# janbruedigam/ConstrainedControl.jl

Hardware: AMD Instinct MI355X
Metric: LQR sim steps/sec (whole node) on N-link cartpole batch (higher is better)
Workload: dtype f64; 1 GPU; lqr_cartpole_n_pendulum N=16 links (17 bodies), hanging-equilibrium LQR, Q=I R=1 horizon 10s, y0~U(-0.5,0.5) phi_i~U(-0.2,0.2); instances_per_gpu=8192, sim_steps=1000, record=True, parallelism=instances sharded x1, lanes_per_instance=32, lds_bytes_per_workgroup=40816, launches_per_rollout=1

## Files before the change

### constrainedcontrol.jl_amd/csrc/cclqr_chain.h

```cpp
#pragma once
#include "cclqr_dev.h"

#if defined(__HIP_DEVICE_COMPILE__)
#define SCHED_FENCE() __builtin_amdgcn_sched_barrier(0)
#else
#define SCHED_FENCE() ((void)0)
#endif
#if defined(__HIP_DEVICE_COMPILE__)
#define LDS_RD(L, i) (*(const volatile __attribute__((address_space(3))) double*)(const __attribute__((address_space(3))) double*)((L) + (i)))
#else
#define LDS_RD(L, i) ((L)[i])
#endif

namespace cclqr {

struct LinkC {
    double m, J[9], p1[3], p2[3], V12[6], qoc[4], axis[3];
    double dtm;
    double sxb, sxa;
    double fric;
    int flags;
    HD bool on() const { return (flags & 1) != 0; }
    HD bool has_a() const { return (flags & 2) != 0; }
    HD bool has_c() const { return (flags & 4) != 0; }
// ... 632 lines not shown
}

struct TriPlanB { TriPlan P; int merge, st; };
HD TriPlanB tri_plan_balanced(int cs, int cn, int st = 1, int fronts = 2) {
    TriPlanB B;
    B.P = tri_plan(0, cn);
    const int rest = cn - 1;
    B.merge = (fronts == 2 && rest > 0 && rest % 2 == 0) ? 1 : 0;
    if (B.merge) { B.P.nA = B.P.nB = rest / 2; B.P.steps = rest / 2; }
    if (fronts == 1) { B.P.nB = 0; B.P.nA = rest; B.P.steps = rest; }
    B.P.cs = cs; B.P.mid = cs + st * B.P.nB; B.st = st;
    return B;
}
HD int tri_scratch_S(const TriPlanB& B, const Lay& Y) { return Y.SJP + 25 * (B.P.cs + B.st); }
HD int tri_scratch_R(const TriPlanB& B, const Lay& Y) { return Y.SPJ + 25 * (B.P.cs + 1); }
struct TriCur {
    int oLL, oQL, oRhs, oTgt, oOut;
    int dblk, dvec;
    int n;
    int imerge, oScr;
    bool isy;
};
HD TriCur tri_cursor(int t, const TriPlanB& B, const Lay& Y) {
    const TriPlan& P = B.P;
    TriCur K;
    const int front = t >> 3, col = t & 7;
    const bool in = t < 16 && col < 6;
    K.n = in ? (front ? P.nB : P.nA) : 0;
    K.isy = col == 5;
    const int st = B.st;
    const int l = front ? P.cs : P.cs + st * (P.cn - 1), q = front ? l + st : l - st;
    const int cc = col < 5 ? col : 0;
    K.dblk = front ? 25 * st : -25 * st;
    K.dvec = K.isy ? (front ? 5 * st : -5 * st) : K.dblk;
    K.oLL = Y.SJJ + 25 * l;
    K.oQL = front ? Y.SJP + 25 * q : Y.SPJ + 25 * (q + 1);
    K.oRhs = K.isy ? Y.R + 5 * l : (front ? Y.SPJ + 25 * (l + 1) : Y.SJP + 25 * l) + 5 * cc;
    K.oTgt = K.isy ? Y.R + 5 * q : Y.SJJ + 25 * q + 5 * cc;
    K.oOut = K.isy ? Y.R + 5 * l : Y.SJJ + 25 * l + 5 * cc;
    K.imerge = (front && B.merge) ? P.nB - 1 : -1;
    K.oScr = K.isy ? tri_scratch_R(B, Y) : tri_scratch_S(B, Y) + 5 * cc;
    return K;
}
HD void lu5_factor(double* A) {
#pragma unroll
    for (int k = 0; k < 5; k++) {
        const double inv = fast_rcp(A[k * 5 + k]);
        A[k * 5 + k] = inv;
#pragma unroll
        for (int i = k + 1; i < 5; i++) {
            const double f = A[i * 5 + k] * inv;
            A[i * 5 + k] = f;
#pragma unroll
            for (int j = k + 1; j < 5; j++) A[i * 5 + j] -= f * A[k * 5 + j];
        }
    }
}
HD bool tri_step(TriCur& K, int i, const double* L, double* tg, double* zy, int* otg, int* oout) {
    if (i >= K.n) return false;
    double lu[25], sql[25];
#pragma unroll
    for (int cI = 0; cI < 5; cI++)
#pragma unroll
        for (int r = 0; r < 5; r++) lu[r * 5 + cI] = LDS_RD(L, K.oLL + 5 * cI + r);
#pragma unroll
    for (int r = 0; r < 5; r++) zy[r] = LDS_RD(L, K.oRhs + r);
    const bool mstep = i == K.imerge;
    double tl[5];
#pragma unroll
    for (int r = 0; r < 5; r++) tl[r] = LDS_RD(L, K.oTgt + r);
#pragma unroll
    for (int r = 0; r < 5; r++) tg[r] = mstep ? 0.0 : tl[r];
#pragma unroll
    for (int e = 0; e < 25; e++) sql[e] = LDS_RD(L, K.oQL + e);
    lu5_factor(lu);
    lu5_solve(lu, zy);
#pragma unroll
    for (int r = 0; r < 5; r++) tg[r] -= sql[r] * zy[0] + sql[5 + r] * zy[1] + sql[10 + r] * zy[2] + sql[15 + r] * zy[3] + sql[20 + r] * zy[4];
    *otg = mstep ? K.oScr : K.oTgt; *oout = K.oOut;
    K.oLL += K.dblk; K.oQL += K.dblk; K.oRhs += K.dvec; K.oTgt += K.dvec; K.oOut += K.dvec;
    return true;
}
HD void tri_step_store(double* L, int otg, int oout, const double* tg, const double* zy) {
#pragma unroll
    for (int r = 0; r < 5; r++) { L[otg + r] = tg[r]; L[oout + r] = zy[r]; }
}
template <bool SCR = true>
HD void ck_tri_mid(int t, const TriPlanB& B, const Lay& Y, double* L) {
    if (t != 0) return;
    const TriPlan& P = B.P;
    double A[25], As[25], b[5], bs[5];
    const int oS = tri_scratch_S(B, Y), oR = tri_scratch_R(B, Y);
#pragma unroll
    for (int cI = 0; cI < 5; cI++)
#pragma unroll
        for (int r = 0; r < 5; r++) A[r * 5 + cI] = LDS_RD(L, Y.SJJ + 25 * P.mid + 5 * cI + r);
#pragma unroll
    for (int cI = 0; cI < 5; cI++)
#pragma unroll
        for (int r = 0; r < 5; r++) As[r * 5 + cI] = SCR ? LDS_RD(L, oS + 5 * cI + r) : 0.0;
#pragma unroll
    for (int i = 0; i < 5; i++) b[i] = LDS_RD(L, Y.R + 5 * P.mid + i);
#pragma unroll
    for (int i = 0; i < 5; i++) bs[i] = SCR ? LDS_RD(L, oR + i) : 0.0;
    const bool merge = SCR && B.merge != 0;
#pragma unroll
    for (int i = 0; i < 5; i++) b[i] = b[i] + (merge ? bs[i] : 0.0);
#pragma unroll
    for (int e = 0; e < 25; e++) A[e] = A[e] + (merge ? As[e] : 0.0);
    lu5_factor(A);
    lu5_solve(A, b);
#pragma unroll
    for (int i = 0; i < 5; i++) L[Y.DL + 5 * P.mid + i] = b[i];
}
HD void ck_tri_back(int t, int j, const TriPlanB& B, const Lay& Y, double* L) {
    const TriPlan& P = B.P;
    const int front = t >> 3, row = t & 7;
    if (t >= 16 || row >= 5) return;
    if (j >= (front ? P.nB : P.nA)) return;
    const int l = front ? P.mid - B.st * (1 + j) : P.mid + B.st * (1 + j);
    const int nbr = front ? l + B.st : l - B.st;
    double z[5], dn[5];
#pragma unroll
    for (int cI = 0; cI < 5; cI++) { z[cI] = LDS_RD(L, Y.SJJ + 25 * l + 5 * cI + row); dn[cI] = LDS_RD(L, Y.DL + 5 * nbr + cI); }
    const double y = LDS_RD(L, Y.R + 5 * l + row);
    L[Y.DL + 5 * l + row] = y - (z[0] * dn[0] + z[1] * dn[1] + z[2] * dn[2] + z[3] * dn[3] + z[4] * dn[4]);
}

HD void tri_step_store_fold(double* L, int otg, int oout, const double* tg, const double* zy, bool last) {
    if (!last) {
#pragma unroll
        for (int r = 0; r < 5; r++) L[otg + r] = tg[r];
    }
#pragma unroll
    for (int r = 0; r < 5; r++) L[oout + r] = zy[r];
}
struct TriBack0 { double z[5], y; int l; bool on; };
HD void ck_tri_back0_load(TriBack0& Q, int t, bool done, const TriPlanB& B, const TriCur& K, const Lay& Y, const double* L) {
    const TriPlan& P = B.P;
    const int front = t >> 3, row = t & 7;
    Q.on = !done && t < 16 && row < 5 && 0 < (front ? P.nB : P.nA);
    Q.l = P.mid + (Q.on ? B.st * (1 - 2 * front) : 0);
    const int rr = row < 5 ? row : 0;
    const bool nostep = P.steps == 0;
    const int o = nostep ? K.oOut : Y.SJJ + 25 * Q.l + rr, d = nostep ? 1 : 5;
#pragma unroll
    for (int cI = 0; cI < 5; cI++) Q.z[cI] = LDS_RD(L, o + d * cI);
    Q.y = LDS_RD(L, Y.R + 5 * Q.l + rr);
}
HD void ck_tri_back0_store(const TriBack0& Q, int t, const Lay& Y, double* L, const double* dn) {
    if (Q.on) L[Y.DL + 5 * Q.l + (t & 7)] = Q.y - (Q.z[0] * dn[0] + Q.z[1] * dn[1] + Q.z[2] * dn[2] + Q.z[3] * dn[3] + Q.z[4] * dn[4]);
}

template <int W>
struct CrLane {
    static const int NS = (11 + W - 1) / W;
    int fl;
    int w;
    int oLL, oPL, oNL;
    int oRhs[NS], oA[NS], oB[NS];
    double z[NS][5];
    HD bool act() const { return (fl & 1) != 0; }
    HD bool has_n() const { return (fl & 2) != 0; }
    HD bool ok(int s) const { return (fl & (4 << s)) != 0; }
    HD int kind(int s) const { const int k = w + W * s; return (k >= 5 ? 1 : 0) + (k >= 10 ? 1 : 0); }
};
#if defined(__HIP_DEVICE_COMPILE__)
#define CR_FLAGS_FRESH(K) asm volatile("" : "+v"((K).fl), "+v"((K).w))
#else
#define CR_FLAGS_FRESH(K) ((void)0)
#endif
template <int W>
HD void cr_setup(CrLane<W>& K, int t, int cs, int n, int st, const Lay& Y, bool skip) {
    const int i = t / W;
    K.w = t - W * i;
    const int nodd = n / 2, idx = 2 * i + 1;
    const bool act = i < nodd && !skip, has_n = idx + 1 < n;
    const int l = act ? cs + st * idx : cs + st, p = l - st, nx = l + st;
    K.oLL = Y.SJJ + 25 * l;
    K.oPL = Y.SPJ + 25 * (p + 1);
    K.oNL = has_n ? Y.SJP + 25 * nx : K.oPL;
    K.fl = (act ? 1 : 0) | (has_n ? 2 : 0);
#pragma unroll
    for (int s = 0; s < CrLane<W>::NS; s++) {
        const int k = K.w + W * s;
        const int T = K.kind(s), cI = k - 5 * T;
        const bool ok = act && k < 11 && (T != 1 || has_n);
        K.fl |= ok ? (4 << s) : 0;
        const int up_l = has_n ? Y.SPJ + 25 * (l + 1) : K.oLL;
        K.oRhs[s] = T == 0 ? Y.SJP + 25 * l + 5 * cI : (T == 1 ? up_l + 5 * cI : Y.R + 5 * l);
        K.oA[s] = T == 0 ? Y.SJJ + 25 * p + 5 * cI : (T == 1 ? K.oPL + 5 * cI : Y.R + 5 * p);
        const int nn = has_n ? nx : p;
        K.oB[s] = T == 0 ? K.oNL + 5 * cI : (T == 1 ? Y.SJJ + 25 * nn + 5 * cI : Y.R + 5 * nn);
        if (!ok) { K.oRhs[s] = K.oLL; K.oA[s] = K.oLL; K.oB[s] = K.oLL; }
    }
}
template <int W>
HD void cr_phase_a(CrLane<W>& K, const double* L, double (*tA)[5]) {
    if (!K.act()) return;
    double lu[25], blk[25];
#pragma unroll
    for (int cI = 0; cI < 5; cI++)
#pragma unroll
        for (int r = 0; r < 5; r++) lu[r * 5 + cI] = LDS_RD(L, K.oLL + 5 * cI + r);
#pragma unroll
    for (int s = 0; s < CrLane<W>::NS; s++)
#pragma unroll
        for (int r = 0; r < 5; r++) K.z[s][r] = LDS_RD(L, K.oRhs[s] + r);
    lu5_factor(lu);
#pragma unroll
    for (int s = 0; s < CrLane<W>::NS; s++) lu5_solve(lu, K.z[s]);
    SCHED_FENCE();
#pragma unroll
    for (int e = 0; e < 25; e++) blk[e] = LDS_RD(L, K.oPL + e);
#pragma unroll
    for (int s = 0; s < CrLane<W>::NS; s++)
#pragma unroll
        for (int r = 0; r < 5; r++) tA[s][r] = LDS_RD(L, K.oA[s] + r);
#pragma unroll
    for (int s = 0; s < CrLane<W>::NS; s++) {
        const double* z = K.z[s];
        const double keep = K.kind(s) != 1 ? 1.0 : 0.0;
#pragma unroll
        for (int r = 0; r < 5; r++) tA[s][r] = keep * tA[s][r] - (blk[r] * z[0] + blk[5 + r] * z[1] + blk[10 + r] * z[2] + blk[15 + r] * z[3] + blk[20 + r] * z[4]);
    }
}
template <int W>
HD void cr_store_a(const CrLane<W>& K, double* L, const double (*tA)[5]) {
#pragma unroll
    for (int s = 0; s < CrLane<W>::NS; s++)
        if (K.ok(s)) {
#pragma unroll
            for (int r = 0; r < 5; r++) { L[K.oRhs[s] + r] = K.z[s][r]; L[K.oA[s] + r] = tA[s][r]; }
        }
}
template <int W>
HD void cr_phase_b(const CrLane<W>& K, const double* L, double (*tB)[5]) {
    if (!(K.act() && K.has_n())) return;
    double blk[25];
#pragma unroll
    for (int s = 0; s < CrLane<W>::NS; s++)
#pragma unroll
        for (int r = 0; r < 5; r++) tB[s][r] = LDS_RD(L, K.oB[s] + r);
#pragma unroll
    for (int e = 0; e < 25; e++) blk[e] = LDS_RD(L, K.oNL + e);
#pragma unroll
    for (int s = 0; s < CrLane<W>::NS; s++) {
        const double* z = K.z[s];
        const double keep = K.kind(s) != 0 ? 1.0 : 0.0;
#pragma unroll
        for (int r = 0; r < 5; r++) tB[s][r] = keep * tB[s][r] - (blk[r] * z[0] + blk[5 + r] * z[1] + blk[10 + r] * z[2] + blk[15 + r] * z[3] + blk[20 + r] * z[4]);
    }
}
template <int W>
HD void cr_store_b(const CrLane<W>& K, double* L, const double (*tB)[5]) {
#pragma unroll
    for (int s = 0; s < CrLane<W>::NS; s++)
        if (K.ok(s) && K.has_n()) {
#pragma unroll
            for (int r = 0; r < 5; r++) L[K.oB[s] + r] = tB[s][r];
        }
}
template <int W>
HD void cr_back(int t, int cs, int n, int st, const Lay& Y, double* L, bool skip) {
    const int i = t / W, w = t - W * i;
    const int idx = 2 * i + 1;
    if (!(i < n / 2) || skip) return;
    const int l = cs + st * idx, p = l - st, nx = l + st;
    const bool has_n = idx + 1 < n;
    double dp[5], dn[5];
#pragma unroll
    for (int cI = 0; cI < 5; cI++) { dp[cI] = LDS_RD(L, Y.DL + 5 * p + cI); const double dnx = LDS_RD(L, Y.DL + 5 * nx + cI); dn[cI] = has_n ? dnx : 0.0; }
    const int oZm = Y.SJP + 25 * l, oZp = has_n ? Y.SPJ + 25 * (l + 1) : oZm;
    double out[(5 + W - 1) / W];
#pragma unroll
    for (int q = 0; q < (5 + W - 1) / W; q++) {
        const int row = w + W * q, rr = row < 5 ? row : 0;
        double acc = LDS_RD(L, Y.R + 5 * l + rr);
#pragma unroll
        for (int cI = 0; cI < 5; cI++) { acc -= LDS_RD(L, oZm + 5 * cI + rr) * dp[cI]; const double zp = LDS_RD(L, oZp + 5 * cI + rr); acc -= (has_n ? zp : 0.0) * dn[cI]; }
        out[q] = acc;
    }
#pragma unroll
    for (int q = 0; q < (5 + W - 1) / W; q++) {
        const int row = w + W * q;
        if (row < 5) L[Y.DL + 5 * l + row] = out[q];
    }
}
#define CR_MIN_LINKS 12

HD Lay make_chain_layout(int nb) {
    Lay L;
    L.S = L.ST = L.LT = L.DS = L.XQ = L.NB = L.DTM = L.G = L.GKB = L.GVA = L.GVB = L.UJ = L.CD = L.SS = 0;
    int o = 0;
    L.SJJ = o; o += 25 * nb; L.SJP = o; o += 25 * nb; L.SPJ = o; o += 25 * nb;
    L.R = o; o += 5 * nb; L.DL = o; o += 5 * nb;
    L.GKA = o; o += GKSZ * nb;
    L.LAM = o; o += 5 * nb;
    L.DINV = o; o += 9 * nb;
    L.D = o; o += 6 * nb;
    L.C = o; o += 6 * nb;
    L.Z = L.SJJ;
    L.DZ = L.SJJ + 13 * nb;
    L.total = o | 1;
    return L;
}
// ... 14 lines not shown
```

### constrainedcontrol.jl_amd/csrc/cclqr_newton.h

```cpp
#pragma once
#include "cclqr_dev.h"

namespace cclqr {

#ifdef CCLQR_PROFILE
enum { PF_CONTROL, PF_FORCES, PF_EVAL_BODY, PF_EVAL_JOINT, PF_EVAL_MAP, PF_SCHUR_W, PF_SCHUR_S, PF_TRI_FWD, PF_TRI_BWD, PF_BODY_SOLVE, PF_TRIAL,
       PF_ACCEPT, PF_IO, PF_NEWTON_ITERS, PF_EVALS, PF_STEPS, PF_ROWS_SKIPPED, PF_N };
static __device__ unsigned long long g_prof[PF_N];
struct Prof {
    unsigned long long t0, acc[PF_N];
    __device__ void start() { for (int i = 0; i < PF_N; i++) acc[i] = 0; t0 = __builtin_readcyclecounter(); }
    __device__ void stamp(int c) { unsigned long long t1 = __builtin_readcyclecounter(); acc[c] += t1 - t0; t0 = t1; }
    __device__ void count(int c, int n = 1) { acc[c] += n; }
    __device__ void flush() { if ((threadIdx.x & 63) == 0) for (int i = 0; i < PF_N; i++) atomicAdd(&g_prof[i], acc[i]); }
};
enum { PF_READ_N = 16 };
static_assert(PF_READ_N == PF_ROWS_SKIPPED && PF_READ_N <= PF_N, "a new counter goes behind the words that two-argument readers receive");
static inline int prof_read(unsigned long long* out, int cap, int reset) {
    int n = cap < PF_N ? cap : PF_N;
    if (!out || n < 0) return -1;
    hipError_t e = hipMemcpyFromSymbol(out, HIP_SYMBOL(g_prof), sizeof(unsigned long long) * n);
    if (e == hipSuccess && reset) { unsigned long long z[PF_N] = {0}; e = hipMemcpyToSymbol(HIP_SYMBOL(g_prof), z, sizeof(z)); }
    return e == hipSuccess ? n : -1;
}
#define PROF_ARG , Prof& prof
#define PROF_PASS , prof
#define STAMP(c) prof.stamp(c)
#define PCOUNT(c) prof.count(c)
#else
#define PROF_ARG
#define PROF_PASS
#define STAMP(c)
#define PCOUNT(c)
#endif

#define NEWTON_EPS 1e-10
#define NEWTON_MAXIT 100
#define LINE_MAXIT 10

struct NewtonStatus { int worst; bool bad, dead; };
__device__ __forceinline__ NewtonStatus status_decode(int carried) {
    return {carried < 0 ? -carried : carried, carried < 0, carried < 0 && carried > -NEWTON_MAXIT};
}
__device__ __forceinline__ int status_encode(int worst, bool bad, bool dead, int carry) {
    return bad ? -((carry && dead && worst >= NEWTON_MAXIT) ? NEWTON_MAXIT - 1 : worst) : worst;
}

template <int N>
__device__ __forceinline__ double dpp_row_ror(double v) {
    int lo = __double2loint(v), hi = __double2hiint(v);
    lo = __builtin_amdgcn_update_dpp(0, lo, 0x120 + N, 0xf, 0xf, true);
    hi = __builtin_amdgcn_update_dpp(0, hi, 0x120 + N, 0xf, 0xf, true);
    return __hiloint2double(hi, lo);
}
template <int CTRL>
__device__ __forceinline__ double dpp_f64(double v) {
    int lo = __double2loint(v), hi = __double2hiint(v);
    lo = __builtin_amdgcn_update_dpp(0, lo, CTRL, 0xf, 0xf, true);
    hi = __builtin_amdgcn_update_dpp(0, hi, CTRL, 0xf, 0xf, true);
    return __hiloint2double(hi, lo);
}
template <int G>
__device__ __forceinline__ double group_sum(double v) {
    if (G == 8) {
        v += dpp_f64<0x141>(v);
        v += dpp_f64<0xB1>(v);
        v += dpp_f64<0x4E>(v);
        return v;
    }
    v += dpp_row_ror<8>(v);
    v += dpp_row_ror<4>(v);
    v += dpp_row_ror<2>(v);
    v += dpp_row_ror<1>(v);
    if (G == 32) v += __shfl_xor(v, 16, 64);
    if (G == 64) {
        int lo = __double2loint(v), hi = __double2hiint(v);
        double r0 = __hiloint2double(__builtin_amdgcn_readlane(hi, 0), __builtin_amdgcn_readlane(lo, 0));
        double r1 = __hiloint2double(__builtin_amdgcn_readlane(hi, 16), __builtin_amdgcn_readlane(lo, 16));
        double r2 = __hiloint2double(__builtin_amdgcn_readlane(hi, 32), __builtin_amdgcn_readlane(lo, 32));
        double r3 = __hiloint2double(__builtin_amdgcn_readlane(hi, 48), __builtin_amdgcn_readlane(lo, 48));
        v = (r0 + r1) + (r2 + r3);
    }
    return v;
}

__device__ __forceinline__ Lay fresh_layout(int nb) {
    asm volatile("" : "+s"(nb));
    return make_layout(nb, 0);
}
#define FRESH_Y fresh_layout(nb)
__device__ __forceinline__ int fresh_lane(int t) {
    asm volatile("" : "+v"(t));
    return t;
}
#define FRESH_T fresh_lane(t)
#define FRESH_PHASE(M, r) asm volatile("" : "+s"(M), "+v"((r).parent), "+v"((r).childl), "+v"((r).rotmask), "+v"((r).type))

template <int G, bool JAC>
__device__ __forceinline__ double eval_point(int t, int nb, const Lay& Y, double* L, LaneRegs& r, const MechDev* M, double dt,
                                             int s_off, double alpha, bool active PROF_ARG) {
    FRESH_PHASE(M, r);
    double part = active ? ph_body_eval<JAC>(FRESH_T, nb, FRESH_Y, L, r, dt, s_off, alpha) : 0.0;
    __syncthreads();
    STAMP(PF_EVAL_BODY);
    FRESH_PHASE(M, r);
    part += active ? ph_joint_eval<JAC>(FRESH_T, nb, FRESH_Y, L, r, dt) : 0.0;
    __syncthreads();
    STAMP(PF_EVAL_JOINT);
    double nrm = sqrt(group_sum<G>(part));
    STAMP(PF_EVAL_MAP);
    PCOUNT(PF_EVALS);
    return nrm;
}

template <int G, bool TREE = false>
__device__ __forceinline__ int newton_solve(int t, int nb, const Lay& Y, double* L, LaneRegs& r, const MechDev* M, double dt, bool valid,
                                            bool* converged PROF_ARG) {
    double normf0 = eval_point<G, true>(t, nb, FRESH_Y, L, r, M, dt, Y.S, 0.0, valid PROF_PASS);
    bool done = !valid, failed = false;
    int its = 0;
    const unsigned long long smask = M->start_mask, emask = M->end_mask;
    const int nchains = M->nchains;
    int s_cur = Y.S, s_try = Y.ST, l_cur = Y.LAM, l_try = Y.LT;
    const int NL = newton_level_groups(G, nb), lg = t / nb, tl = t - lg * nb;
    for (int iter = 1; iter <= NEWTON_MAXIT; iter++) {
        if (!__any(!done)) break;
        PCOUNT(PF_NEWTON_ITERS);
        FRESH_PHASE(M, r);
        if (TREE) {
            if (!done) ph_schur_s_tree(FRESH_T, G, nb, FRESH_Y, L, M);
            __syncthreads();
            STAMP(PF_SCHUR_S);
            FRESH_PHASE(M, r);
            {
                const Lay Ye = FRESH_Y;
                const int te = FRESH_T;
                for (int l = nb - 1; l >= 0; l--) {
                    if (!done) ph_tree_elim(te, l, Ye, L, M);
                    __syncthreads();
                }
            }
            STAMP(PF_TRI_FWD);
            FRESH_PHASE(M, r);
            {
                const Lay Yb = FRESH_Y;
                const int tb = FRESH_T;
                for (int l = 0; l < nb; l++) {
                    if (!done) ph_tree_back(tb, l, Yb, L, M);
                    __syncthreads();
                }
            }
            STAMP(PF_TRI_BWD);
            FRESH_PHASE(M, r);
            if (!done) ph_body_solve_tree(FRESH_T, G, nb, FRESH_Y, L, M);
            __syncthreads();
            STAMP(PF_BODY_SOLVE);
        } else {
        if (!done) ph_schur_s(FRESH_T, G, nb, FRESH_Y, L, smask);
        __syncthreads();
        STAMP(PF_SCHUR_S);
        for (int c = 0; c < nchains; c++) {
            const TriPlan P = tri_plan(M->chain_start[c], M->chain_len[c]);
            for (int i = 0; i < P.steps; i++) {
                double lu[5];
                int l = 0;
                bool act = !done && ph_tri_elim(FRESH_T, i, P, FRESH_Y, L, lu, &l);
                if (act) ph_tri_store(FRESH_T, l, FRESH_Y, L, lu);
                __syncthreads();
            }
            STAMP(PF_TRI_FWD);
            if (!done) ph_tri_mid(FRESH_T, P, FRESH_Y, L);
            __syncthreads();
            for (int j = 0; j < P.steps; j++) {
                if (!done) ph_tri_back(FRESH_T, j, P, FRESH_Y, L);
                __syncthreads();
            }
            STAMP(PF_TRI_BWD);
        }
        FRESH_PHASE(M, r);
        if (!done) ph_body_solve(FRESH_T, G, nb, FRESH_Y, L, emask);
        __syncthreads();
        STAMP(PF_BODY_SOLVE);
        }
        double alpha = 1.0, normf1 = 0.0, nd = 0.0;
        bool ls_done = done, jac_ok = true;
        {
            double pd = ls_done ? 0.0 : ph_trial(FRESH_T, G, nb, FRESH_Y, L, alpha, s_cur, s_try, l_cur, l_try);
            nd = sqrt(group_sum<G>(pd));
            __syncthreads();
            STAMP(PF_TRIAL);
            double nf = eval_point<G, true>(t, nb, FRESH_Y, L, r, M, dt, s_try, alpha, !ls_done PROF_PASS);
            if (!ls_done) {
                normf1 = nf;
                if (!(normf1 > normf0)) ls_done = true;
            }
            __syncthreads();
        }
        for (int lv = 1; lv <= LINE_MAXIT; lv += NL) {
            if (!__any(!ls_done)) break;
            FRESH_PHASE(M, r);
            const int mylv = lv + lg;
            const bool lane_on = !ls_done && lg < NL && mylv <= LINE_MAXIT;
            const double a_l = ldexp(1.0, -mylv);
            const Lay V = level_layout(FRESH_Y, nb, lg < NL ? lg : 0);
            if (lane_on) ph_trial_level(fresh_lane(tl), nb, FRESH_Y, V, L, a_l, s_cur, l_cur);
            __syncthreads();
            STAMP(PF_TRIAL);
            double part = lane_on ? ph_body_eval<false>(fresh_lane(tl), nb, V, L, r, dt, V.ST, a_l) : 0.0;
            __syncthreads();
            STAMP(PF_EVAL_BODY);
            part += lane_on ? ph_joint_eval<false>(fresh_lane(tl), nb, V, L, r, dt) : 0.0;
            __syncthreads();
            STAMP(PF_EVAL_JOINT);
// ... 39 lines not shown
```

### constrainedcontrol.jl_amd/csrc/rollout_chain.hip

```cpp
#include "cclqr_chain.h"
#include "cclqr_internal.h"
#include "cclqr_newton.h"
#include "cclqr_rollout_step.h"

namespace cclqr {

__device__ __forceinline__ double wave_from_prev(double v) {
    int lo = __double2loint(v), hi = __double2hiint(v);
    lo = __builtin_amdgcn_update_dpp(0, lo, 0x138, 0xf, 0xf, true);
    hi = __builtin_amdgcn_update_dpp(0, hi, 0x138, 0xf, 0xf, true);
    return __hiloint2double(hi, lo);
}
__device__ __forceinline__ double wave_from_next(double v) {
    int lo = __double2loint(v), hi = __double2hiint(v);
    lo = __builtin_amdgcn_update_dpp(0, lo, 0x130, 0xf, 0xf, true);
    hi = __builtin_amdgcn_update_dpp(0, hi, 0x130, 0xf, 0xf, true);
    return __hiloint2double(hi, lo);
}
template <int N>
__device__ __forceinline__ void from_prev(const double* in, double* out) {
#pragma unroll
    for (int i = 0; i < N; i++) out[i] = wave_from_prev(in[i]);
}
template <int N>
__device__ __forceinline__ void from_next(const double* in, double* out) {
#pragma unroll
    for (int i = 0; i < N; i++) out[i] = wave_from_next(in[i]);
}

__device__ __forceinline__ void ck_tri_mid_regs(int t, bool done, const TriPlanB& B, const TriCur& K, const Lay& Y, const double* L, const double* tg, double* dl, TriBack0& Q) {
    const TriPlan& P = B.P;
    ck_tri_back0_load(Q, t, done, B, K, Y, L);
    double m[5];
    const bool ran = K.n == P.steps;
#pragma unroll
    for (int r = 0; r < 5; r++) m[r] = ran ? tg[r] : 0.0;
    if (P.steps == 0) {
        asm volatile("");
        const bool f0 = (t & 8) == 0;
#pragma unroll
        for (int r = 0; r < 5; r++) m[r] = f0 ? Q.z[r] : 0.0;
    }
#pragma unroll
    for (int r = 0; r < 5; r++) m[r] = m[r] + dpp_row_ror<8>(m[r]);
    double A[25];
#pragma unroll
    for (int i = 0; i < 5; i++) {
        A[i * 5 + 0] = dpp_f64<0x150>(m[i]); A[i * 5 + 1] = dpp_f64<0x151>(m[i]); A[i * 5 + 2] = dpp_f64<0x152>(m[i]);
        A[i * 5 + 3] = dpp_f64<0x153>(m[i]); A[i * 5 + 4] = dpp_f64<0x154>(m[i]);
        dl[i] = dpp_f64<0x155>(m[i]);
    }
    lu5_factor(A);
    lu5_solve(A, dl);
}

__device__ __forceinline__ auto swap_rows_b32(unsigned first, unsigned second) { return __builtin_amdgcn_permlane16_swap(first, second, false, false); }
template <bool KEEP, int N>
__device__ __forceinline__ void from_row_below(double* v, bool keep) {
    double cp[N];
#pragma unroll
    for (int i = 0; i < N; i++) { cp[i] = v[i]; asm volatile("" : "+v"(cp[i])); }
#pragma unroll
    for (int i = 0; i < N; i++) {
        const auto a = swap_rows_b32((unsigned)__double2loint(cp[i]), (unsigned)__double2loint(v[i]));
        const auto b = swap_rows_b32((unsigned)__double2hiint(cp[i]), (unsigned)__double2hiint(v[i]));
        const unsigned lo = KEEP ? (keep ? a[1] : a[0]) : a[0], hi = KEEP ? (keep ? b[1] : b[0]) : b[0];
        v[i] = __hiloint2double((int)hi, (int)lo);
    }
}
template <int G, int NBP, int KL> struct SchurSplit { static const bool ON = G == 32 && NBP <= 17 && KL == 1, R0 = NBP == 17; };
template <int NBP>
__device__ __forceinline__ void schur_split_setup(LinkC& c, int t, const MechDev* M, int nb) {
    const int l = t & 15;
    const bool help = t >= 16 && !c.on();
    double sl = c.sxb;
    from_row_below<false, 1>(&sl, false);
    if (help) schur_split_helper(c, l < nb && M->childl[l] >= 0, sl);
}
template <bool R0>
__device__ __forceinline__ void schur_split_take(const LinkC& c, int t, double (*wXT)[3], double (*wPB)[3]) {
    const bool keep = R0 && t >= 16 && !c.help();
#pragma unroll
    for (int r = 0; r < 3; r++) from_row_below<R0, 3>(wXT[r], keep);
#pragma unroll
    for (int r = 0; r < 5; r++) from_row_below<R0, 3>(wPB[r], keep);
}

template <int G, bool JAC, int KL = 1, int SP = 0>
__device__ __forceinline__ double chain_eval(LinkC& c, LinkS& S, int t, const Lay& Y, double* L, double alpha, bool active, bool inst_on, bool rows, double dt, const SubSel& Q PROF_ARG) {
    double part = 0.0;
    double NB[9], g[5], xq[7];
    const bool store_dinv = JAC && __any(rows);
    LINK_FLAGS_FRESH(c);
#pragma unroll
    for (int k = 0; k < 7; k++) xq[k] = S.z[k];
    if (active) {
        double cf[6], sv[6], cTR[6], DINV[9];
#pragma unroll
        for (int k = 0; k < 6; k++) { cf[k] = L[Y.C + 6 * t + k] - alpha * S.cd[k]; sv[k] = S.s[k] - alpha * S.ds[k]; cTR[k] = L[Y.D + 6 * t + k]; }
        part = ck_body_eval<JAC>(c, S.z, sv, cf, cTR, cTR + 3, dt, xq, S.d, DINV, NB);
        if (KL > 1 && !c.prim()) part = 0.0;
        if (store_dinv && (KL == 1 || c.prim())) {
#pragma unroll
            for (int k = 0; k < 9; k++) L[Y.DINV + 9 * t + k] = DINV[k];
        }
    }
    STAMP(PF_EVAL_BODY);
    double pxq[7], pNB[9];
    from_prev<7>(xq, pxq);
    if (JAC) from_prev<9>(NB, pNB);
    if (!c.has_a()) {
#pragma unroll
        for (int i = 0; i < 7; i++) pxq[i] = (i == 3) ? 1.0 : 0.0;
    }
    if (JAC && KL > 1) {
        constexpr int NR = SubRows<KL>::NR;
        double gs[NR], sXT[NR][3], sPB[NR][3], sPA[NR][3];
        if (active) {
            joint_eval_rows<KL>(c, Q, pxq, pxq + 3, xq, xq + 3, pNB, NB, gs, sXT, sPB, sPA);
#pragma unroll
            for (int i = 0; i < NR; i++) part += gs[i] * gs[i];
        }
        STAMP(PF_EVAL_JOINT);
        LINK_FLAGS_FRESH(c);
        if (__any(rows)) {
            double pd[6];
            from_prev<6>(S.d, pd);
            ck_schur_rows_sub<KL, (KL == 3)>(c, Q, t, active, Y, L, gs, sXT, sPB, sPA, S.d, pd);
        } else {
            PCOUNT(PF_ROWS_SKIPPED);
        }
        STAMP(PF_SCHUR_S);
    } else {
        double wXT[3][3], wPB[5][3], wPA[5][3];
        if constexpr (JAC && SP != 0) {
#pragma unroll
            for (int r = 0; r < 3; r++)
#pragma unroll
                for (int k = 0; k < 3; k++) asm volatile("" : "=v"(wXT[r][k]));
#pragma unroll
            for (int r = 0; r < 5; r++)
#pragma unroll
                for (int k = 0; k < 3; k++) asm volatile("" : "=v"(wPB[r][k]));
        }
        if (active) {
            joint_eval_sparse<JAC>(c, pxq, pxq + 3, xq, xq + 3, pNB, NB, g, wXT, wPB, wPA);
            if (KL == 1) {
#pragma unroll
                for (int i = 0; i < 5; i++) part += g[i] * g[i];
            } else {
                double pj = 0.0;
#pragma unroll
                for (int i = 0; i < 5; i++) pj += g[i] * g[i];
                part += c.prim() ? pj : 0.0;
            }
        }
        STAMP(PF_EVAL_JOINT);
        LINK_FLAGS_FRESH(c);
        if (JAC) {
            if (__any(rows)) {
                double pd[6];
                from_prev<6>(S.d, pd);
                if constexpr (SP != 0) {
                    schur_split_take<SP == 2>(c, t, wXT, wPB);
                    ck_schur_rows_split<SP == 2>(c, t, active, inst_on, Y, L, wXT, wPB, wPA, g, S.d, pd);
                } else {
                    ck_schur_rows(c, t, active, Y, L, wXT, wPB, wPA, g, S.d, pd);
                }
            } else {
                PCOUNT(PF_ROWS_SKIPPED);
            }
            STAMP(PF_SCHUR_S);
        }
    }
    const double nrm = sqrt(group_sum<G>(part));
    STAMP(PF_EVAL_MAP);
    PCOUNT(PF_EVALS);
    return nrm;
}

template <int G, int KL = 1>
__device__ __forceinline__ void chain_eval2(LinkC& c, const TrialIn& T, const double* Lc, int t, const Lay& Y, double a1, double a2, bool active, double dt,
                                            double& n1, double& n2) {
    double part1 = 0.0, part2 = 0.0, xq1[7], xq2[7];
    LINK_FLAGS_FRESH(c);
#pragma unroll
    for (int k = 0; k < 7; k++) { xq1[k] = T.z[k]; xq2[k] = T.z[k]; }
    if (active) {
        double cf1[6], cf2[6], sv1[6], sv2[6], cTR[6], d1[6], d2[6];
#pragma unroll
        for (int k = 0; k < 6; k++) {
            const double cc = Lc[Y.C + 6 * t + k];
            cTR[k] = Lc[Y.D + 6 * t + k];
            cf1[k] = cc - a1 * T.cd[k]; cf2[k] = cc - a2 * T.cd[k];
            sv1[k] = T.s[k] - a1 * T.ds[k]; sv2[k] = T.s[k] - a2 * T.ds[k];
        }
        part1 = ck_body_eval<false>(c, T.z, sv1, cf1, cTR, cTR + 3, dt, xq1, d1, nullptr, nullptr);
        part2 = ck_body_eval<false>(c, T.z, sv2, cf2, cTR, cTR + 3, dt, xq2, d2, nullptr, nullptr);
    }
    double p1[7], p2[7];
    from_prev<7>(xq1, p1);
    from_prev<7>(xq2, p2);
    if (!c.has_a()) {
#pragma unroll
        for (int i = 0; i < 7; i++) { p1[i] = (i == 3) ? 1.0 : 0.0; p2[i] = p1[i]; }
    }
    if (active) {
        double g1[5], g2[5];
        joint_eval_sparse<false>(c, p1, p1 + 3, xq1, xq1 + 3, nullptr, nullptr, g1, (double(*)[3]) nullptr, (double(*)[3]) nullptr, (double(*)[3]) nullptr);
        joint_eval_sparse<false>(c, p2, p2 + 3, xq2, xq2 + 3, nullptr, nullptr, g2, (double(*)[3]) nullptr, (double(*)[3]) nullptr, (double(*)[3]) nullptr);
#pragma unroll
        for (int i = 0; i < 5; i++) { part1 += g1[i] * g1[i]; part2 += g2[i] * g2[i]; }
    }
    if (KL > 1 && !c.prim()) { part1 = 0.0; part2 = 0.0; }
    n1 = sqrt(group_sum<G>(part1));
    n2 = sqrt(group_sum<G>(part2));
}

template <int G, int KL = 1>
__device__ __forceinline__ double chain_eval1(LinkC& c, const TrialIn& T, const double* Lc, int t, const Lay& Y, double a1, bool active, double dt) {
    double part1 = 0.0, xq1[7];
    LINK_FLAGS_FRESH(c);
#pragma unroll
// ... 123 lines not shown
        const CtrlRows rows = ctrl_step_rows(C, k, gi, nz, ne);
        const bool gate = rows.gate;
        const GlobalD Kp = global_table(C->K) + rows.K + t;
        const GlobalD Fp = C->Fd ? global_table(C->Fd) + rows.Fd : (GlobalD)0;
        double grav = M->g;
        unsigned long long zd_base = C->zd;
        asm volatile("" : "+s"(zd_base));
        double* const traj_out = ap->traj;
        if (traj_out) {
            if (c.live() && (KL == 1 || c.prim())) {
                LANE_INT_FRESH(plan);
                const int ub = plan >> 24;
#pragma unroll
                for (int i = 0; i < 7; i++) L[Y.Z + 13 * ub + i] = S.z[i];
#pragma unroll
                for (int i = 0; i < 6; i++) L[Y.Z + 13 * ub + 7 + i] = S.s[i];
            }
        }
        STAMP(PF_IO);
        double uj = 0.0;
        double zf[13], za[13];
#pragma unroll
        for (int i = 0; i < 7; i++) zf[i] = S.z[i];
#pragma unroll
        for (int i = 0; i < 6; i++) zf[7 + i] = S.s[i];
        from_prev<7>(zf, za);
        if (EXTRA) from_prev<6>(zf + 7, za + 7);
        if (!c.has_a()) {
#pragma unroll
            for (int i = 0; i < 13; i++) za[i] = (i == 3) ? 1.0 : 0.0;
        }
        if (gate) {
            if (c.live()) {
                double dz[12], zdv[13];
                const GlobalD zp = global_table(zd_base) + rows.zd + 13 * tl;
#pragma unroll
                for (int i = 0; i < 13; i++) zdv[i] = zp[i];
                ck_control_error(zf, zdv, dz);
                if (KL == 1 || c.prim()) {
#pragma unroll
                    for (int i = 0; i < 12; i++) L[Y.DZ + 12 * tl + i] = dz[i];
                }
                if (EXTRA && (C->flags & CtrlHot::FRIC) && c.has_fric()) uj = ck_friction(c, zf, za);
            }
        }
        WAVE_HANDOVER();
        if (gate) {
            constexpr int NE = GainRows<G, NBP>::NE;
            double unoise = 0.0;
            if (EXTRA == 3) {
                if (C->flags & CtrlHot::NOISE) unoise = C->noise_scale * philox_normal_dev(C->noise_key0, (unsigned long long)gi, k);
            } else if (EXTRA) {
                const double* noise = ap->noise;
                if ((C->flags & CtrlHot::NOISE) && c.valid() && noise) unoise = C->noise_scale * noise[(size_t)inst * ap->noise_stride + (k - 1)];
            }
            double dzv[NE];
            int tf = t;
            asm volatile("" : "+v"(tf));
#pragma unroll
            for (int q = 0; q < NE; q++) { const int e = tf + q * G; dzv[q] = (c.valid() && e < ne) ? L[Y.DZ + e] : 0.0; }
            feedback_inputs<G, NBP, EXTRA>(C, Kp, Fp, mu, ne, dzv, unoise, tc, uj);
        }
        STAMP(PF_CONTROL);
        asm volatile("" : "+v"(grav));
        if (traj_out) {
            if (c.valid()) {
                int kr = kk, nzr = nz;
                asm volatile("" : "+s"(kr), "+s"(nzr));
                double* dst = traj_out + ((size_t)inst * ap->steps + kr) * nzr;
                int e0 = t;
                asm volatile("" : "+v"(e0));
                for (int e = e0; e < nz; e += G) dst[e] = L[Y.Z + e];
            }
        }
        STAMP(PF_IO);
        if (EXTRA == 2 && (C->flags & CtrlHot::PID)) {
            if (c.live() && CT->pid_on[tl]) uj += ck_pid(c, zf, za, CT->pid_P[tl], CT->pid_I[tl], CT->pid_D[tl], CT->pid_goal[tl], dt, k == 1, pid_int, pid_last);
        }
        STAMP(PF_CONTROL);
        LINK_FLAGS_FRESH(c);
        {
            double F[3], tau[3], W6[6], cW6[6];
            ck_joint_wrench(c, uj, zf + 3, za + 3, F, tau, W6, W6 + 3);
            from_next<6>(W6, cW6);
            if (c.has_c()) {
#pragma unroll
                for (int i = 0; i < 3; i++) { F[i] += cW6[i]; tau[i] += cW6[3 + i]; }
            }
            double cTR[6];
            ck_step_invariants(c, zf, F, tau, dt, grav, cTR, cTR + 3);
            double gk[5], kXT[3][3], kPB[5][3], kPA[5][3], lam[5];
            joint_eval_sparse<true>(c, za, za + 3, zf, zf + 3, nullptr, nullptr, gk, kXT, kPB, kPA);
#pragma unroll
            for (int i = 0; i < 5; i++) lam[i] = L[Y.LAM + 5 * tl + i];
            if (c.live() && (KL == 1 || c.prim())) {
                gk_store(tl, Y, L, kXT, kPB, kPA);
#pragma unroll
                for (int i = 0; i < 6; i++) L[Y.D + 6 * tl + i] = cTR[i];
            }
            double own[6], par[6], cpar[6];
            jac_t_apply(c, kXT, kPB, kPA, lam, own, par);
            from_next<6>(par, cpar);
#pragma unroll
            for (int i = 0; i < 6; i++) S.cd[i] = 0.0;
            if (c.live() && (KL == 1 || c.prim())) {
#pragma unroll
                for (int i = 0; i < 6; i++) L[Y.C + 6 * tl + i] = own[i] + (c.has_c() ? cpar[i] : 0.0);
            }
        }
        WAVE_HANDOVER();

        STAMP(PF_FORCES);
        PCOUNT(PF_STEPS);
        const bool go = c.valid() && !c.dead();
        bool done = !go, failed = false;
        int its = 0;
        double normf0 = 0.0;
        LANE_INT_FRESH(plan);
        const int nchains = chain_plan_count(__builtin_amdgcn_readfirstlane(plan));
        bool need_jac = !done;
        for (int iter = 1; iter <= NEWTON_MAXIT; iter++) {
            if (__any(need_jac)) {
                const double nf = chain_eval<G, true, KL, SP>(c, S, tl, Y, L, 0.0, c.live() && need_jac, need_jac, need_jac, dt, Q PROF_PASS);
                if (iter == 1) normf0 = nf;
            }
            WAVE_HANDOVER();
            if (!__any(!done)) break;
            PCOUNT(PF_NEWTON_ITERS);
            const bool active = c.live() && !done;
            for (int ci = 0; ci < nchains; ci++) {
                const int pw = __builtin_amdgcn_readlane(plan, ci);
                const int cs = chain_plan_start(pw), cn = chain_plan_len(pw);
                constexpr int CRW = 4;
                constexpr bool CR = G == 32 && NBP <= 17;
                const bool cr = CR && cn >= CR_MIN_LINKS;
                if (CR && cr) {
                    CrLane<CRW> CK;
                    double tc[CrLane<CRW>::NS][5];
                    cr_setup<CRW>(CK, t, cs, cn, 1, Y, done);
                    CR_FLAGS_FRESH(CK);
                    cr_phase_a<CRW>(CK, L, tc);
                    CR_FLAGS_FRESH(CK);
                    cr_store_a<CRW>(CK, L, tc);
                    WAVE_HANDOVER();
                    CR_FLAGS_FRESH(CK);
                    cr_phase_b<CRW>(CK, L, tc);
                    CR_FLAGS_FRESH(CK);
                    cr_store_b<CRW>(CK, L, tc);
                    WAVE_HANDOVER();
                }
                STAMP(PF_SCHUR_W);
                const TriPlanB PB = cr ? tri_plan_balanced(cs, (cn + 1) / 2, 2) : tri_plan_balanced(cs, cn, 1, G >= 16 ? 2 : 1);
                const TriPlan& P = PB.P;
                TriCur K = tri_cursor(t, PB, Y);
                if (done) K.n = 0;
                if constexpr (G >= 16) {
                    double tg[5] = {0.0, 0.0, 0.0, 0.0, 0.0}, dlm[5];
                    for (int i = 0; i < P.steps; i++) {
                        double zy[5];
                        int otg = 0, oout = 0;
                        int left = P.steps - 1 - i;
                        LANE_INT_FRESH(left);
                        if (tri_step(K, i, L, tg, zy, &otg, &oout)) tri_step_store_fold(L, otg, oout, tg, zy, left == 0);
                        WAVE_HANDOVER();
                    }
                    STAMP(PF_TRI_FWD);
                    TriBack0 B0;
                    ck_tri_mid_regs(t, done, PB, K, Y, L, tg, dlm, B0);
                    ck_tri_back0_store(B0, t, Y, L, dlm);
                    WAVE_HANDOVER();
                    for (int j = 1; j < P.steps; j++) {
                        if (!done) ck_tri_back(t, j, PB, Y, L);
                        WAVE_HANDOVER();
                    }
                    if (!done && t == 0) {
#pragma unroll
                        for (int i = 0; i < 5; i++) L[Y.DL + 5 * P.mid + i] = dlm[i];
                    }
                    WAVE_HANDOVER();
                } else {
                    for (int i = 0; i < P.steps; i++) {
                        double tg[5], zy[5];
                        int otg = 0, oout = 0;
                        if (tri_step(K, i, L, tg, zy, &otg, &oout)) tri_step_store(L, otg, oout, tg, zy);
                        WAVE_HANDOVER();
                    }
                    STAMP(PF_TRI_FWD);
                    if (!done) ck_tri_mid<false>(t, PB, Y, L);
                    WAVE_HANDOVER();
                    for (int j = 0; j < P.steps; j++) {
                        if (!done) ck_tri_back(t, j, PB, Y, L);
                        WAVE_HANDOVER();
                    }
                }
                if (CR && cr) {
                    cr_back<CRW>(t, cs, cn, 1, Y, L, done);
                    WAVE_HANDOVER();
                }
                STAMP(PF_TRI_BWD);
            }
            double nd;
            LINK_FLAGS_FRESH(c);
            {
                double own[6], par[6], cpar[6], dl[5], pdn = 0.0;
#pragma unroll
                for (int r = 0; r < 5; r++) dl[r] = L[Y.DL + 5 * tl + r];
                gk_t_apply<true>(c, tl, Y, L, dl, own, par);
                from_next<6>(par, cpar);
                if (active) {
                    double DINV[9];
#pragma unroll
                    for (int i = 0; i < 9; i++) DINV[i] = L[Y.DINV + 9 * tl + i];
#pragma unroll
                    for (int i = 0; i < 6; i++) S.cd[i] = own[i] + (c.has_c() ? cpar[i] : 0.0);
                    ck_body_solve(c, S.d, S.cd, DINV, S.ds);
#pragma unroll
                    for (int i = 0; i < 6; i++) pdn += S.ds[i] * S.ds[i];
#pragma unroll
                    for (int i = 0; i < 5; i++) pdn += dl[i] * dl[i];
                    if (KL > 1 && !c.prim()) pdn = 0.0;
                }
                nd = sqrt(group_sum<G>(pdn));
            }
            WAVE_HANDOVER();
            STAMP(PF_BODY_SOLVE);
            double alpha = 1.0, normf1 = 0.0;
            const bool want_rows = !done && !(normf0 < NEWTON_EPS && nd < NEWTON_EPS);
            bool ls_done = done, jac_ok = __any(want_rows);
            {
                const double nf = chain_eval<G, true, KL, SP>(c, S, tl, Y, L, 1.0, active, !done, want_rows, dt, Q PROF_PASS);
                if (!ls_done) {
                    normf1 = nf;
                    if (!(normf1 > normf0)) ls_done = true;
                }
            }
            if (G == 32) {
                for (int lv = 1; lv <= LINE_MAXIT;) {
                    if (!__any(!ls_done)) break;
                    const bool mine = !ls_done;
                    const bool other = __shfl_xor(mine ? 1 : 0, 32, 64) != 0;
                    const bool solo = ap->plants != nullptr;
                    const bool helping = !mine && other && !solo;
                    TrialIn T;
#pragma unroll
                    for (int i = 0; i < 7; i++) T.z[i] = S.z[i];
#pragma unroll
                    for (int i = 0; i < 6; i++) { T.s[i] = S.s[i]; T.ds[i] = S.ds[i]; T.cd[i] = S.cd[i]; }
                    if (mine != other) {
#pragma unroll
                        for (int i = 0; i < 7; i++) { const double o = other_half(S.z[i]); T.z[i] = helping ? o : T.z[i]; }
#pragma unroll
                        for (int i = 0; i < 6; i++) {
                            const double o1 = other_half(S.s[i]), o2 = other_half(S.ds[i]), o3 = other_half(S.cd[i]);
                            T.s[i] = helping ? o1 : T.s[i]; T.ds[i] = helping ? o2 : T.ds[i]; T.cd[i] = helping ? o3 : T.cd[i];
                        }
                    }
                    const double* Lc = helping ? lds + (1 - grp) * Y.total : L;
                    const int l0 = helping ? lv + 2 : lv;
                    double n1, n2;
                    chain_eval2<G, KL>(c, T, Lc, tl, Y, ldexp(1.0, -l0), ldexp(1.0, -(l0 + 1)), c.on() && (mine || helping) && l0 <= LINE_MAXIT, dt, n1, n2);
                    PCOUNT(PF_EVALS);
                    const double h1 = other_half(n1), h2 = other_half(n2);
                    if (mine) {
                        const double cand[4] = {n1, n2, h1, h2};
#pragma unroll
                        for (int i = 0; i < 4; i++) {
                            const int l = lv + i;
                            if (!ls_done && l <= LINE_MAXIT && (i < 2 || !(other || solo))) {
                                normf1 = cand[i]; alpha = ldexp(1.0, -l); jac_ok = false;
                                if (!(cand[i] > normf0) || l == LINE_MAXIT) ls_done = true;
                            }
                        }
                    }
                    lv += (solo || (mine && other)) ? 2 : 4;
                }
            } else {
                constexpr int NG = 64 / G;
                for (int lv = 1; lv <= LINE_MAXIT;) {
                    if (!__any(!ls_done)) break;
                    const bool mine = !ls_done;
                    const unsigned long long heads = __ballot(mine && t == 0);
                    const bool solo = ap->plants != nullptr;
                    const int count = solo ? NG : __builtin_popcountll(heads);
                    const int per = NG / count;
                    const int kq = grp % count, off = grp / count;
                    unsigned long long hm = heads;
                    for (int i = 0; i < kq; i++) hm &= hm - 1;
                    const int src = solo ? grp : __builtin_ctzll(hm) / G;
                    int myrank = 0;
                    for (int g2 = 0; g2 < NG; g2++) myrank += (g2 < grp && ((heads >> (g2 * G)) & 1ull)) ? 1 : 0;
                    const int l0 = lv + off;
                    const bool work = off < per && l0 <= LINE_MAXIT;
                    const int fa = (src * G + t) * 4;
                    TrialIn T;
#pragma unroll
                    for (int i = 0; i < 7; i++) T.z[i] = S.z[i];
#pragma unroll
                    for (int i = 0; i < 6; i++) { T.s[i] = S.s[i]; T.ds[i] = S.ds[i]; T.cd[i] = S.cd[i]; }
                    if (count < NG) {
#pragma unroll
                        for (int i = 0; i < 7; i++) T.z[i] = lane_fetch(S.z[i], fa);
#pragma unroll
                        for (int i = 0; i < 6; i++) { T.s[i] = lane_fetch(S.s[i], fa); T.ds[i] = lane_fetch(S.ds[i], fa); T.cd[i] = lane_fetch(S.cd[i], fa); }
                    }
                    const double nf = chain_eval1<G, KL>(c, T, lds + src * Y.total, tl, Y, ldexp(1.0, -l0), c.on() && work, dt);
                    PCOUNT(PF_EVALS);
                    if (count == NG) {
                        if (mine) {
                            normf1 = nf; alpha = ldexp(1.0, -lv); jac_ok = false;
// ... 141 lines not shown
```

Before: 29.71 million instance-steps/s.

## Map block-tridiagonal sweep to 16-lane rows with DPP broadcasts

For the 32-lane chain path, the block-tridiagonal forward sweep gets a new lane mapping. Each 5x5 block row now lives in a 16-lane DPP row, and the LU pivot block is assembled with row_newbcast DPP broadcasts instead of being re-read from LDS. The Schur update uses inline-asm v_fmac_f64_dpp, and the back substitution and middle solve are reworked for the 16-lane row layout. The aim is fewer LDS reads and shorter dependency chains per sweep step. The cost is hand-written asm with s_nop hazard handling and an extra code path that must match the old one numerically.

After: 29.98 million instance-steps/s, median of 6. About the same (+0.9%).

```diff
diff --git a/constrainedcontrol.jl_amd/csrc/cclqr_chain.h b/constrainedcontrol.jl_amd/csrc/cclqr_chain.h
--- a/constrainedcontrol.jl_amd/csrc/cclqr_chain.h
+++ b/constrainedcontrol.jl_amd/csrc/cclqr_chain.h
@@ -808,6 +808,84 @@
     if (Q.on) L[Y.DL + 5 * Q.l + (t & 7)] = Q.y - (Q.z[0] * dn[0] + Q.z[1] * dn[1] + Q.z[2] * dn[2] + Q.z[3] * dn[3] + Q.z[4] * dn[4]);
 }
 
+HD TriCur tri_cursor_rows(int t, const TriPlanB& B, const Lay& Y) {
+    const int front = t >> 4, col = t & 15;
+    TriCur K = tri_cursor(col < 6 ? 8 * front + col : 6, B, Y);
+    K.oQL += col < 5 ? 5 * col : 0;
+    return K;
+}
+HD void tri_rows_first(const TriCur& K, const double* L, double* tg) {
+#pragma unroll
+    for (int r = 0; r < 5; r++) tg[r] = LDS_RD(L, K.oOut + r);
+}
+HD void tri_rows_load(const TriCur& K, int i, const double* L, const double* tg, double* zy, double* tn, double* q) {
+#pragma unroll
+    for (int r = 0; r < 5; r++) zy[r] = LDS_RD(L, K.oRhs + r);
+#pragma unroll
+    for (int r = 0; r < 5; r++) zy[r] = K.isy ? tg[r] : zy[r];
+    const bool mstep = i == K.imerge;
+    double tl[5];
+#pragma unroll
+    for (int r = 0; r < 5; r++) tl[r] = LDS_RD(L, K.oTgt + r);
+#pragma unroll
+    for (int r = 0; r < 5; r++) tn[r] = mstep ? 0.0 : tl[r];
+#pragma unroll
+    for (int r = 0; r < 5; r++) q[r] = LDS_RD(L, K.oQL + r);
+}
+HD void tri_rows_solve(double* lu, double* zy) {
+    lu5_factor(lu);
+    lu5_solve(lu, zy);
+}
+HD void tri_rows_update(double* tn, const double* s, const double* zy) {
+#pragma unroll
+    for (int r = 0; r < 5; r++) tn[r] -= s[r] * zy[0] + s[5 + r] * zy[1] + s[10 + r] * zy[2] + s[15 + r] * zy[3] + s[20 + r] * zy[4];
+}
+HD void tri_rows_finish(TriCur& K, int i, int kn, double* tg, const double* tn, int* otg, int* oout) {
+    LANE_INT_FRESH(kn);
+    const bool work = i < kn;
+#pragma unroll
+    for (int r = 0; r < 5; r++) tg[r] = work ? tn[r] : tg[r];
+    *otg = K.oTgt; *oout = K.oOut;
+    const int db = work ? K.dblk : 0, dv = work ? K.dvec : 0;
+    K.oQL += db; K.oRhs += dv; K.oTgt += dv; K.oOut += dv;
+}
+HD bool tri_rows_keep(int i, int kn, int left) { return i + 1 == kn && left != 0; }
+HD void tri_rows_store(double* L, int otg, int oout, const double* tg, const double* zy, bool keep) {
+    if (keep) {
+#pragma unroll
+        for (int r = 0; r < 5; r++) L[otg + r] = tg[r];
+    }
+#pragma unroll
+    for (int r = 0; r < 5; r++) L[oout + r] = zy[r];
+}
+HD bool tri_rows_mid_mine(const TriCur& K, const TriPlan& P, int t) { return K.n == P.steps && (P.steps != 0 || (t & 16) == 0); }
+HD void ck_tri_back0_load_rows(TriBack0& Q, int t, bool done, const TriPlanB& B, const Lay& Y, const double* L) {
+    const TriPlan& P = B.P;
+    const int front = t >> 4, row = t & 15;
+    Q.on = !done && row < 5 && 0 < (front ? P.nB : P.nA);
+    Q.l = P.mid + (Q.on ? B.st * (1 - 2 * front) : 0);
+    const int rr = row < 5 ? row : 0;
+#pragma unroll
+    for (int cI = 0; cI < 5; cI++) Q.z[cI] = LDS_RD(L, Y.SJJ + 25 * Q.l + rr + 5 * cI);
+    Q.y = LDS_RD(L, Y.R + 5 * Q.l + rr);
+}
+HD void ck_tri_back0_store_rows(const TriBack0& Q, int t, const Lay& Y, double* L, const double* dn) {
+    if (Q.on) L[Y.DL + 5 * Q.l + (t & 15)] = Q.y - (Q.z[0] * dn[0] + Q.z[1] * dn[1] + Q.z[2] * dn[2] + Q.z[3] * dn[3] + Q.z[4] * dn[4]);
+}
+HD void ck_tri_back_rows(int t, int j, const TriPlanB& B, const Lay& Y, double* L) {
+    const TriPlan& P = B.P;
+    const int front = t >> 4, row = t & 15;
+    if (row >= 5) return;
+    if (j >= (front ? P.nB : P.nA)) return;
+    const int l = front ? P.mid - B.st * (1 + j) : P.mid + B.st * (1 + j);
+    const int nbr = front ? l + B.st : l - B.st;
+    double z[5], dn[5];
+#pragma unroll
+    for (int cI = 0; cI < 5; cI++) { z[cI] = LDS_RD(L, Y.SJJ + 25 * l + 5 * cI + row); dn[cI] = LDS_RD(L, Y.DL + 5 * nbr + cI); }
+    const double y = LDS_RD(L, Y.R + 5 * l + row);
+    L[Y.DL + 5 * l + row] = y - (z[0] * dn[0] + z[1] * dn[1] + z[2] * dn[2] + z[3] * dn[3] + z[4] * dn[4]);
+}
+
 template <int W>
 struct CrLane {
     static const int NS = (11 + W - 1) / W;
diff --git a/constrainedcontrol.jl_amd/csrc/cclqr_newton.h b/constrainedcontrol.jl_amd/csrc/cclqr_newton.h
--- a/constrainedcontrol.jl_amd/csrc/cclqr_newton.h
+++ b/constrainedcontrol.jl_amd/csrc/cclqr_newton.h
@@ -59,6 +59,10 @@
     lo = __builtin_amdgcn_update_dpp(0, lo, CTRL, 0xf, 0xf, true);
     hi = __builtin_amdgcn_update_dpp(0, hi, CTRL, 0xf, 0xf, true);
     return __hiloint2double(hi, lo);
+}
+template <int CTRL>
+__device__ __forceinline__ double dpp_b64(double v) {
+    return __builtin_amdgcn_update_dpp(0.0, v, CTRL, 0xf, 0xf, true);
 }
 template <int G>
 __device__ __forceinline__ double group_sum(double v) {
diff --git a/constrainedcontrol.jl_amd/csrc/rollout_chain.hip b/constrainedcontrol.jl_amd/csrc/rollout_chain.hip
--- a/constrainedcontrol.jl_amd/csrc/rollout_chain.hip
+++ b/constrainedcontrol.jl_amd/csrc/rollout_chain.hip
@@ -69,6 +69,71 @@
     }
 }
 template <int G, int NBP, int KL> struct SchurSplit { static const bool ON = G == 32 && NBP <= 17 && KL == 1, R0 = NBP == 17; };
+template <int G, int NBP> struct SweepRows { static const bool ON = G == 32 && NBP <= 17; };
+
+#define SWEEP_BC(k) " row_newbcast:" #k " row_mask:0xf bank_mask:0xf\n\t"
+__device__ __forceinline__ void tri_rows_update_dpp(double* tn, const double* q, const double* zy) {
+    double a0 = dpp_b64<0x150>(q[0]) * zy[0], a1 = dpp_b64<0x150>(q[1]) * zy[0], a2 = dpp_b64<0x150>(q[2]) * zy[0], a3 = dpp_b64<0x150>(q[3]) * zy[0],
+           a4 = dpp_b64<0x150>(q[4]) * zy[0];
+    asm volatile("s_nop 4\n\t"
+                 "v_fmac_f64_dpp %0, %5, %10" SWEEP_BC(1) "v_fmac_f64_dpp %1, %6, %10" SWEEP_BC(1) "v_fmac_f64_dpp %2, %7, %10" SWEEP_BC(1)
+                 "v_fmac_f64_dpp %3, %8, %10" SWEEP_BC(1) "v_fmac_f64_dpp %4, %9, %10" SWEEP_BC(1)
+                 "v_fmac_f64_dpp %0, %5, %11" SWEEP_BC(2) "v_fmac_f64_dpp %1, %6, %11" SWEEP_BC(2) "v_fmac_f64_dpp %2, %7, %11" SWEEP_BC(2)
+                 "v_fmac_f64_dpp %3, %8, %11" SWEEP_BC(2) "v_fmac_f64_dpp %4, %9, %11" SWEEP_BC(2)
+                 "v_fmac_f64_dpp %0, %5, %12" SWEEP_BC(3) "v_fmac_f64_dpp %1, %6, %12" SWEEP_BC(3) "v_fmac_f64_dpp %2, %7, %12" SWEEP_BC(3)
+                 "v_fmac_f64_dpp %3, %8, %12" SWEEP_BC(3) "v_fmac_f64_dpp %4, %9, %12" SWEEP_BC(3)
+                 "v_fmac_f64_dpp %0, %5, %13" SWEEP_BC(4) "v_fmac_f64_dpp %1, %6, %13" SWEEP_BC(4) "v_fmac_f64_dpp %2, %7, %13" SWEEP_BC(4)
+                 "v_fmac_f64_dpp %3, %8, %13" SWEEP_BC(4) "v_fmac_f64_dpp %4, %9, %13" SWEEP_BC(4)
+                 : "+v"(a0), "+v"(a1), "+v"(a2), "+v"(a3), "+v"(a4)
+                 : "v"(q[0]), "v"(q[1]), "v"(q[2]), "v"(q[3]), "v"(q[4]), "v"(zy[1]), "v"(zy[2]), "v"(zy[3]), "v"(zy[4]));
+    tn[0] = tn[0] - a0; tn[1] = tn[1] - a1; tn[2] = tn[2] - a2; tn[3] = tn[3] - a3; tn[4] = tn[4] - a4;
+}
+__device__ __forceinline__ void tri_step_rows(TriCur& K, int i, int kn, const double* L, double* tg, double* zy, int* otg, int* oout) {
+    if (i >= CCLQR_MAXL) return;
+    double lu[25], tn[5], q[5];
+#pragma unroll
+    for (int r = 0; r < 5; r++) {
+        lu[r * 5 + 0] = dpp_b64<0x150>(tg[r]); lu[r * 5 + 1] = dpp_b64<0x151>(tg[r]); lu[r * 5 + 2] = dpp_b64<0x152>(tg[r]);
+        lu[r * 5 + 3] = dpp_b64<0x153>(tg[r]); lu[r * 5 + 4] = dpp_b64<0x154>(tg[r]);
+    }
+    tri_rows_load(K, i, L, tg, zy, tn, q);
+    tri_rows_solve(lu, zy);
+#if defined(__HIP_DEVICE_COMPILE__)
+    tri_rows_update_dpp(tn, q, zy);
+#else
+    double s[25];
+#pragma unroll
+    for (int r = 0; r < 5; r++) {
+        s[r] = dpp_b64<0x150>(q[r]); s[5 + r] = dpp_b64<0x151>(q[r]); s[10 + r] = dpp_b64<0x152>(q[r]);
+        s[15 + r] = dpp_b64<0x153>(q[r]); s[20 + r] = dpp_b64<0x154>(q[r]);
+    }
+    tri_rows_update(tn, s, zy);
+#endif
+    tri_rows_finish(K, i, kn, tg, tn, otg, oout);
+}
+__device__ __forceinline__ void ck_tri_mid_regs_rows(int t, bool done, const TriPlanB& B, const TriCur& K, const Lay& Y, const double* L, const double* tg, double* dl, TriBack0& Q) {
+    const TriPlan& P = B.P;
+    ck_tri_back0_load_rows(Q, t, done, B, Y, L);
+    double m[5], cp[5];
+    const bool mine = tri_rows_mid_mine(K, P, t);
+#pragma unroll
+    for (int r = 0; r < 5; r++) { m[r] = mine ? tg[r] : 0.0; cp[r] = m[r]; asm volatile("" : "+v"(cp[r])); }
+#pragma unroll
+    for (int r = 0; r < 5; r++) {
+        const auto a = swap_rows_b32((unsigned)__double2loint(cp[r]), (unsigned)__double2loint(m[r]));
+        const auto b = swap_rows_b32((unsigned)__double2hiint(cp[r]), (unsigned)__double2hiint(m[r]));
+        m[r] = __hiloint2double((int)b[0], (int)a[0]) + __hiloint2double((int)b[1], (int)a[1]);
+    }
+    double A[25];
+#pragma unroll
+    for (int i = 0; i < 5; i++) {
+        A[i * 5 + 0] = dpp_f64<0x150>(m[i]); A[i * 5 + 1] = dpp_f64<0x151>(m[i]); A[i * 5 + 2] = dpp_f64<0x152>(m[i]);
+        A[i * 5 + 3] = dpp_f64<0x153>(m[i]); A[i * 5 + 4] = dpp_f64<0x154>(m[i]);
+        dl[i] = dpp_f64<0x155>(m[i]);
+    }
+    lu5_factor(A);
+    lu5_solve(A, dl);
+}
 template <int NBP>
 __device__ __forceinline__ void schur_split_setup(LinkC& c, int t, const MechDev* M, int nb) {
     const int l = t & 15;
@@ -498,9 +563,36 @@
                 STAMP(PF_SCHUR_W);
                 const TriPlanB PB = cr ? tri_plan_balanced(cs, (cn + 1) / 2, 2) : tri_plan_balanced(cs, cn, 1, G >= 16 ? 2 : 1);
                 const TriPlan& P = PB.P;
-                TriCur K = tri_cursor(t, PB, Y);
+                TriCur K = SweepRows<G, NBP>::ON ? tri_cursor_rows(t, PB, Y) : tri_cursor(t, PB, Y);
                 if (done) K.n = 0;
-                if constexpr (G >= 16) {
+                if constexpr (SweepRows<G, NBP>::ON) {
+                    double tg[5], dlm[5];
+                    tri_rows_first(K, L, tg);
+                    for (int i = 0; i < P.steps; i++) {
+                        double zy[5];
+                        int otg = 0, oout = 0;
+                        int left = P.steps - 1 - i;
+                        LANE_INT_FRESH(left);
+                        const int kn = K.n;
+                        tri_step_rows(K, i, kn, L, tg, zy, &otg, &oout);
+                        if (i < kn) tri_rows_store(L, otg, oout, tg, zy, tri_rows_keep(i, kn, left));
+                        WAVE_HANDOVER();
+                    }
+                    STAMP(PF_TRI_FWD);
+                    TriBack0 B0;
+                    ck_tri_mid_regs_rows(t, done, PB, K, Y, L, tg, dlm, B0);
+                    ck_tri_back0_store_rows(B0, t, Y, L, dlm);
+                    WAVE_HANDOVER();
+                    for (int j = 1; j < P.steps; j++) {
+                        if (!done) ck_tri_back_rows(t, j, PB, Y, L);
+                        WAVE_HANDOVER();
+                    }
+                    if (!done && t == 0) {
+#pragma unroll
+                        for (int i = 0; i < 5; i++) L[Y.DL + 5 * P.mid + i] = dlm[i];
+                    }
+                    WAVE_HANDOVER();
+                } else if constexpr (G >= 16) {
                     double tg[5] = {0.0, 0.0, 0.0, 0.0, 0.0}, dlm[5];
                     for (int i = 0; i < P.steps; i++) {
                         double zy[5];
```
